# RomanJuranek/waldboost

Measured on AMD Instinct MI355X. Metric: candidate windows/s, 1080p grad_hist pyramid, 128-stage depth-2 cascade, higher is better.
Workload: dtype u8 image, f64/f32 channel arithmetic, f32 scores; 1 GPU; BASELINE configs[1]: 1920x1080 uint8, shrink=2 n_per_oct=8 smooth=1 grad_hist, window (12,12,4), 128-stage depth-2 cascade, 1 image(s)/step/GPU; batch_per_gpu=1, levels=64, windows_per_image=3045278, launch=hipGraph replay per step, only=all, channels_in_hbm=uint8 threshold ranks of the cascade (WB_DTYPE_RANK8), streams=4, pool=4, full=False, warm=1668 untimed steps right before the timed ones (--warm-ms 50), cascade_kernel=model-specialised (hiprtc at model load, 0.9 s incl. cache lookup), collective=none

## Files before the change

### waldboost_amd/csrc/wb_channels.hip

```cpp
#include <stdlib.h>
#include <type_traits>

#include "wb_common.h"

namespace {

struct ChanArgs {
    const void *img;
    const void *oct;
    int64_t img_stride, oct_stride;
    const WbLevel *levels;
    const WbTile *tiles;
    const uint32_t *minmax;
    const WbTap *taps;
    int n_oct;
    void *chn;
    int64_t chn_stride;
    double cs[4], sn[4];
    float chi, clo;
    float c2hi, c2lo;
    double tri[11];
    float gm_eps;
    int src_int;
    int dbg;
    uint8_t *rank;
    int64_t rank_stride;
    const WbTilePatch *patches;
    const uint4 *rank_lut;
    int rank_iters;
    float rank_k[4], rank_b[4];
    int rank_wide;
};

#ifdef WB_CASC_STAMPS
#define WB_CSTAMP_SLOTS 8
#define WB_CSTAMP_WGS (1 << 17)
__device__ unsigned long long g_chan_stamps[WB_CSTAMP_WGS * WB_CSTAMP_SLOTS];
#define WB_CSTAMP(k)                                                                                      \
    do {                                                                                                  \
        unsigned long long _wg = (unsigned long long)blockIdx.y * gridDim.x + blockIdx.x;                 \
        if (threadIdx.x == 0 && _wg < WB_CSTAMP_WGS)                                                      \
            g_chan_stamps[_wg * WB_CSTAMP_SLOTS + (k)] = __builtin_amdgcn_s_memrealtime();                \
    } while (0)
#else
#define WB_CSTAMP(k) do {} while (0)
#endif

#ifndef WB_CHAN_UR
#define WB_CHAN_UR 8
#endif
#ifndef WB_CHAN_S4_BYTES
#define WB_CHAN_S4_BYTES 1
#endif
#ifndef WB_CHAN_S4_WAVES
#define WB_CHAN_S4_WAVES (WB_CHAN_S4_BYTES ? 5 : 3)
#endif
#ifndef WB_CHAN_S4_TV
#define WB_CHAN_S4_TV 30
#endif
typedef WbTap Tap;

__device__ inline double lane_f64(double v, int k) {
    const long long b = __double_as_longlong(v);
    const unsigned lo = (unsigned)__builtin_amdgcn_readlane((int)(unsigned)b, k);
    const unsigned hi = (unsigned)__builtin_amdgcn_readlane((int)(unsigned)(b >> 32), k);
    return __longlong_as_double((long long)(((unsigned long long)hi << 32) | lo));
}

typedef const __attribute__((address_space(3))) unsigned char *LdsBytePtr;
__device__ inline uint8_t lds_byte_apart(const unsigned char *p) {
    LdsBytePtr q = (LdsBytePtr)p;
    asm volatile("" : "+v"(q));
    return *q;
}
typedef const volatile __attribute__((address_space(3))) unsigned char *LdsVolBytePtr;
__device__ __forceinline__ uint8_t lds_byte_vol(const unsigned char *patch, int off) {
    return *((LdsVolBytePtr)patch + off);
}
typedef const volatile __attribute__((address_space(3))) uint16_t *LdsVolU16Ptr;
__device__ __forceinline__ uint32_t lds_u16_vol(const unsigned char *base, int off) {
    return *(LdsVolU16Ptr)((LdsVolBytePtr)base + off);
}

__device__ inline double resample_f64(double v00, double v01, double v10, double v11, const Tap &tr, const Tap &tc) {
    double t = (v00 * tr.w0) * tc.w0;
    t = t + (v01 * tr.w0) * tc.w1;
    t = t + (v10 * tr.w1) * tc.w0;
    t = t + (v11 * tr.w1) * tc.w1;
    return t;
}

template <typename T> struct Src;
template <> struct Src<uint8_t> {
    static constexpr bool kFastResample = true;
    static constexpr float kEps = 2.5e-4f;
    static __device__ bool fast(float v00, float v01, float v10, float v11, float wr0, float wr1, float wc0, float wc1,
                                float &out) {
        float top = __builtin_fmaf(v01, wc1, v00 * wc0), bot = __builtin_fmaf(v11, wc1, v10 * wc0);
        return fast_rows(top, bot, wr0, wr1, out);
    }
    static __device__ bool fast_rows(float top, float bot, float wr0, float wr1, float &out) {
        float t = hold(__builtin_fmaf(bot, wr1, hold(top * wr0)));
        float fl = floorf(t), fr = hold(t - fl);
        out = fl;
        return fabsf(hold(fr - 0.5f)) <= 0.5f - kEps;
    }
    static __device__ __forceinline__ float hold(float v) {
        asm volatile("" : "+v"(v));
        return v;
    }
    static __device__ double lo(uint32_t k) { return (double)k; }
    static __device__ float finish(double t, double mn, double mx, int) {
        t = fmin(fmax(t, mn), mx);
        return (float)(int)t;
    }
    static __device__ bool taps_finite(uint8_t, uint8_t, uint8_t) { return true; }
    static __device__ float hpass(float a, float b, float c) { return __builtin_fmaf(b, 2.0f, a + c); }
    static __device__ float dpass(float lo, float, float hi) { return lo - hi; }
};
template <> struct Src<float> {
    static constexpr bool kFastResample = false;
    static __device__ bool fast(float, float, float, float, float, float, float, float, float &) { return false; }
    static __device__ bool fast_rows(float, float, float, float, float &) { return false; }
    static __device__ double lo(uint32_t k) { return (double)wb_key_f32(k); }
    static __device__ float finish(double t, double mn, double mx, int) {
        const float f = (float)t, lo = (float)mn, hi = (float)mx;
        if (lo != lo || hi != hi) return __builtin_nanf("");
        return f < lo ? lo : (f > hi ? hi : f);
    }
    static __device__ bool taps_finite(float a, float b, float c) { return fabsf(a) < INFINITY && fabsf(b) < INFINITY && fabsf(c) < INFINITY; }
    static __device__ float hpass(float a, float b, float c) {
        return (float)((double)b * 2.0 + ((double)a + (double)c));
    }
    static __device__ float dpass(float lo, float mid, float hi) { return (float)((double)mid * 0.0 + ((double)lo - (double)hi)); }
};

template <> struct Src<double> {
    static constexpr bool kFastResample = false;
    static __device__ bool fast(float, float, float, float, float, float, float, float, float &) { return false; }
    static __device__ bool fast_rows(float, float, float, float, float &) { return false; }
    static __device__ double lo(unsigned long long k) {
        const unsigned long long b = (k >> 63) ? (k & 0x7fffffffffffffffull) : ~k;
        return __longlong_as_double((long long)b);
    }
    static __device__ float finish(double t, double mn, double mx, int src_int) {
        if (mn != mn || mx != mx) return __builtin_nanf("");
        t = t < mn ? mn : (t > mx ? mx : t);
        switch (src_int) {
            case WB_CAST_TRUNC: t = trunc(t); break;
            case WB_CAST_BOOL: t = t != 0.0 ? 1.0 : 0.0; break;
            case WB_CAST_F16: t = wb_round_f16(t); break;
        }
        return (float)t;
    }
    static __device__ bool taps_finite(double a, double b, double c) { return fabs(a) < INFINITY && fabs(b) < INFINITY && fabs(c) < INFINITY; }
    static __device__ float hpass(float a, float b, float c) { return Src<float>::hpass(a, b, c); }
    static __device__ float dpass(float lo, float mid, float hi) { return Src<float>::dpass(lo, mid, hi); }
};

template <typename T> __device__ inline void clip_range(const ChanArgs &a, int b, int oct, double &mn, double &mx) {
    if constexpr (sizeof(T) == 8) {
        const unsigned long long *mm = reinterpret_cast<const unsigned long long *>(a.minmax) + ((int64_t)b * a.n_oct + oct) * 2;
        mn = Src<T>::lo(~mm[0]);
        mx = Src<T>::lo(mm[1]);
    } else {
        const uint32_t *mm = a.minmax + ((int64_t)b * a.n_oct + oct) * 2;
        mn = Src<T>::lo(~mm[0]);
        mx = Src<T>::lo(mm[1]);
    }
}

struct F4 {
    float x, y, z, w;
};

__device__ inline float scalar_only(float v) {
    asm volatile("" : "+v"(v));
    return v;
}

__device__ inline double smooth_top(double a, double b, double c) { return __builtin_fma(2.0, b, a) + c; }
__device__ inline double smooth_mid(double s, double d, double e, double f) {
    return __builtin_fma(2.0, f, __builtin_fma(4.0, e, __builtin_fma(2.0, d, s)));
}
__device__ inline float smooth_bot(double s, double g, double h, double i) { return (float)((__builtin_fma(2.0, h, s + g) + i) * 0.0625); }
__device__ inline float smooth9(double a, double b, double c, double d, double e, double f, double g, double h, double i) {
    return smooth_bot(smooth_mid(smooth_top(a, b, c), d, e, f), g, h, i);
}

__device__ inline void project_f64(float gx, float gy, const ChanArgs &a, float *out) {
    double gxd = (double)gx, gyd = (double)gy;
#pragma unroll
    for (int k = 0; k < 4; ++k) {
        float val = (float)(gxd * a.cs[k] - gyd * a.sn[k]);
        out[k] = fmaxf(fabsf(val), 0.0f);
    }
}

__device__ inline void project_int(float gx, float gy, const ChanArgs &a, float *out) {
    const float d1 = fabsf(gx - gy), d3 = fabsf(gx + gy), ax = fabsf(gx);
    const double g = (double)gx;
    const float tiny = fabsf((float)(g * a.cs[1] - g * a.sn[1]));
    const float o1 = __builtin_fmaf(d1, a.chi, d1 * a.clo), o3 = __builtin_fmaf(d3, a.chi, d3 * a.clo);
    out[0] = ax;
    out[1] = d1 == 0.0f ? tiny : o1;
    out[2] = gy == 0.0f ? __builtin_fmaf(ax, a.c2hi, ax * a.c2lo) : fabsf(gy);
    out[3] = d3 == 0.0f ? tiny : o3;
}

constexpr float kSinHi = 0x1.6a09e6p-1f;
constexpr float kSinLo = (float)(0x1.6a09e667f3bccp-1 - (double)kSinHi);
__device__ inline void project_ordinary(float gx, float gy, const ChanArgs &, float *out) {
    const float d1 = gx - gy, d3 = gx + gy;
    out[0] = fabsf(gx);
    out[1] = fabsf(scalar_only(__builtin_fmaf(d1, kSinHi, scalar_only(d1 * kSinLo))));
    out[2] = fabsf(gy);
    out[3] = fabsf(scalar_only(__builtin_fmaf(d3, kSinHi, scalar_only(d3 * kSinLo))));
}

template <int S_, int TU_, int TV_, bool SMOOTH_, int NT_ = 256> struct TileGeom {
    static constexpr int S = S_, TU = TU_, TV = TV_, NT = NT_, NW = NT_ / 64;
    static constexpr bool SMOOTH = SMOOTH_;
    static constexpr int HS = SMOOTH ? 1 : 0;
    static constexpr int SU = TU + 2 * HS, SV = TV + 2 * HS;
    static constexpr int RH = S * SU + 2, RW = S * SV + 2;
    static constexpr int P = S + 2;
    static constexpr int PROWS = S == 2 ? (TU == 16 ? 74 : 2 * RH - 8) : 2 * RH + 4;
    static constexpr int PPITCH = S == 4 ? 2 * RW + 12 : (S == 2 && TU != 16) ? 256 : ((SU * SV * 16) / PROWS) & ~3;
    static_assert(S == 4 || PROWS * PPITCH <= SU * SV * 16, "the source patch shares the shrunk tile's memory");
    static_assert(PPITCH % 4 == 0, "patch rows are written as dwords");
    static constexpr int SH_BYTES = SU * SV * 16;
    static constexpr int PATCH_BYTES = PROWS * PPITCH;
};

__host__ __device__ inline int reflect_index(int i, int n) {
    const int period = 2 * n;
    i %= period;
    if (i < 0) i += period;
    return i >= n ? period - 1 - i : i;
}

template <bool REFLECT> __host__ __device__ __forceinline__ int tile_coord(int i, int n) {
    if constexpr (REFLECT)
        return reflect_index(i, n);
    else
        return i < 0 ? 0 : (i > n - 1 ? n - 1 : i);
}

template <bool REFLECT> __host__ __device__ __forceinline__ void tile_coord_range(int lo, int hi, int n, int &lo_out, int &hi_out) {
    if constexpr (!REFLECT) {
        lo_out = tile_coord<false>(lo, n);
        hi_out = tile_coord<false>(hi, n);
    } else if (lo >= 0 && hi < n) {
        lo_out = lo;
        hi_out = hi;
    } else if (lo < -n || hi >= 2 * n || (lo < 0 && hi >= n)) {
        lo_out = 0;
        hi_out = n - 1;
    } else if (lo < 0) {
        lo_out = hi < 0 ? -1 - hi : 0;
        hi_out = hi < 0 ? -1 - lo : (hi > -1 - lo ? hi : -1 - lo);
    } else {
        hi_out = lo >= n ? 2 * n - 1 - lo : n - 1;
        lo_out = lo >= n ? 2 * n - 1 - hi : (lo < 2 * n - 1 - hi ? lo : 2 * n - 1 - hi);
    }
}

template <typename G, bool REFLECT>
__host__ __device__ __forceinline__ bool tile_patch_extent(const WbLevel &L, int ry0, int rx0, int rh, int &r_lo, int &c_lo, int &nrow,
                                                           int &nbyte) {
    int yf, yl, xf, xl;
    tile_coord_range<REFLECT>(ry0, ry0 + rh - 1, L.nh, yf, yl);
    tile_coord_range<REFLECT>(rx0, rx0 + G::RW - 1, L.nw, xf, xl);
    const bool ident = (L.src_h == L.nh) && (L.src_w == L.nw);
    const bool strict = !ident && L.src_h > L.nh && L.src_w > L.nw;
    auto first_tap = [](int k, double step) { return (int)floor(((double)k + 0.5) * step - 0.5); };
    r_lo = first_tap(yf, L.sy);
    c_lo = first_tap(xf, L.sx);
    const int r_hi = first_tap(yl, L.sy) + 1, c_hi = first_tap(xl, L.sx) + 1;
    nrow = r_hi - r_lo + 1;
    nbyte = c_hi - c_lo + 1;
    return strict && nrow + 1 <= G::PROWS && nbyte + 8 <= G::PPITCH;
}

template <typename RT, int RW> struct RPitch { static constexpr int value = sizeof(RT) == 1 ? ((RW + 3) & ~3) : RW; };

#ifndef WB_CHAN_RB
#define WB_CHAN_RB 2
#endif
__host__ __device__ constexpr int wb_strip_rows(int rh, int nw) { return WB_CHAN_RB * ((rh + nw * WB_CHAN_RB - 1) / (nw * WB_CHAN_RB)); }

template <typename T, typename G, bool REFLECT = false, typename RT = float>
__device__ __forceinline__ void resample_tile(const ChanArgs &a, const WbLevel &L, const T *src, const double mn,
                                              const double mx, const int ry0, const int rx0, const int rh, RT *R,
                                              unsigned char *uni, float4 *rowtab, const int tid) {
    static_assert(sizeof(RT) == 4 || sizeof(T) == 1, "byte R holds uint8 pixels");
    constexpr int RP = RPitch<RT, G::RW>::value;
    auto rput = [&](int idx, float v) {
        if constexpr (sizeof(RT) == 1) R[idx] = (RT)(int)v; else R[idx] = v;
    };
    constexpr int RH = G::RH, RW = G::RW, PPITCH = G::PPITCH, NT = G::NT, NW = G::NW;
    const Tap *__restrict__ rtap = a.taps + L.tap_off;
    const Tap *__restrict__ ctap = rtap + L.nh;
    constexpr int NCS = RW / 64, MAINW = NCS * 64, LEFT = RW - MAINW;
    const int lane = tid & 63, wave = __builtin_amdgcn_readfirstlane(tid >> 6);
    const bool ident = (L.src_h == L.nh) && (L.src_w == L.nw);
    if constexpr (sizeof(T) == 1) {
        constexpr int RWD = (RW + 3) / 4;
        if (ident && ry0 >= 0 && ry0 + RH <= L.nh && rx0 >= 0 && rx0 + 4 * RWD <= L.nw) {
            static_assert(RW % 2 == 0, "pixel pairs");
            typedef uint32_t __attribute__((aligned(1))) u32u;
            constexpr int NE = RH * RWD, PER = (NE + NT - 1) / NT;
            uint32_t v[PER];
            int at[PER];
#pragma unroll
            for (int i = 0; i < PER; ++i) {
                int e = tid + NT * i;
                e = e < NE ? e : NE - 1;
                const int k = e / RWD, d = e - k * RWD;
                v[i] = *reinterpret_cast<const u32u *>(src + (int64_t)(ry0 + k) * L.src_w + rx0 + 4 * d);
                at[i] = k * RP + 4 * d;
            }
#pragma unroll
            for (int i = 0; i < PER; ++i) {
                if constexpr (sizeof(RT) == 1) {
                    *reinterpret_cast<uint32_t *>(R + at[i]) = v[i];
                } else {
                    float2 *dst = reinterpret_cast<float2 *>(R + at[i]);
                    dst[0] = make_float2((float)(v[i] & 0xffu), (float)((v[i] >> 8) & 0xffu));
                    if (at[i] % RW + 2 < RW) dst[1] = make_float2((float)((v[i] >> 16) & 0xffu), (float)(v[i] >> 24));
                }
            }
            WB_CSTAMP(1);
            WB_CSTAMP(2);
            WB_CSTAMP(3);
            return;
        }
    }
    bool staged = false;
    int r_lo = 0, c_lo = 0;
    Tap tcs[NCS], trl, tleft;
    trl.i0 = trl.i1 = 0; trl.w0 = trl.w1 = 0.0;
    tleft = trl;
#pragma unroll
    for (int c = 0; c < NCS; ++c) tcs[c] = trl;
    if constexpr (sizeof(T) == 1) {
        int nrow, nbyte;
        if (a.patches) {
            const WbTilePatch tp = a.patches[blockIdx.x];
            r_lo = tp.r_lo;
            c_lo = tp.c_lo;
            nrow = tp.rows;
            nbyte = tp.bytes;
            staged = nrow != 0;
        } else {
            staged = tile_patch_extent<G, REFLECT>(L, ry0, rx0, rh, r_lo, c_lo, nrow, nbyte);
            r_lo = __builtin_amdgcn_readfirstlane(r_lo);
            c_lo = __builtin_amdgcn_readfirstlane(c_lo);
            nrow = __builtin_amdgcn_readfirstlane(nrow);
            nbyte = __builtin_amdgcn_readfirstlane(nbyte);
        }
        WB_CSTAMP(1);
#pragma unroll
        for (int c = 0; c < NCS; ++c) {
            const int x = tile_coord<REFLECT>(rx0 + lane + 64 * c, L.nw);
            tcs[c] = ctap[x];
        }
        {
            static_assert(wb_strip_rows(RH, NW) <= 64, "one lane per row of the strip");
            const int RS = wb_strip_rows(rh, NW);
            const int kl = wave * RS + lane;
            const int ly = tile_coord<REFLECT>(ry0 + (kl < rh ? kl : rh - 1), L.nh);
            trl = rtap[ly];
            const int lx = tile_coord<REFLECT>(rx0 + MAINW + (lane < LEFT ? lane : 0), L.nw);
            tleft = ctap[lx];
        }
        if (staged) {
            constexpr int DWP = PPITCH / 4;
            const int ndw = (nbyte + 1 + 3) / 4;
            uint32_t *pw = reinterpret_cast<uint32_t *>(uni);
            constexpr int UR = WB_CHAN_UR;
            const int wv = __builtin_amdgcn_readfirstlane(tid >> 6), ln = tid & 63;
            for (int dw0 = 0; dw0 < ndw; dw0 += 64) {
                int dw = dw0 + ln;
                dw = dw < ndw ? dw : ndw - 1;
                const int voff = 4 * dw;
                const uint64_t origin = reinterpret_cast<uint64_t>(src + (int64_t)r_lo * L.src_w + c_lo);
                const uint64_t origin_u = ((uint64_t)(uint32_t)__builtin_amdgcn_readfirstlane((int)(uint32_t)(origin >> 32)) << 32) |
                                          (uint32_t)__builtin_amdgcn_readfirstlane((int)(uint32_t)origin);
                const __amdgpu_buffer_rsrc_t rsrc = __builtin_amdgcn_make_buffer_rsrc(reinterpret_cast<void *>(origin_u), 0, 0x7fffffff, 0x00020000);
                for (int r0 = wv; r0 < nrow; r0 += NW * UR) {
                    uint32_t v[UR];
                    int rr[UR];
#pragma unroll
                    for (int k = 0; k < UR; ++k) {
                        rr[k] = r0 + NW * k < nrow ? r0 + NW * k : nrow - 1;
                        v[k] = __builtin_amdgcn_raw_buffer_load_b32(rsrc, voff, rr[k] * L.src_w, 0);
                    }
#pragma unroll
                    for (int k = 0; k < UR; ++k) pw[rr[k] * DWP + dw] = v[k];
                }
            }
            {
                const int RS = wb_strip_rows(rh, NW);
                const int kl = wave * RS + lane;
                if (lane < RS && kl < rh) rowtab[kl] = make_float4(__int_as_float((trl.i0 - r_lo) * PPITCH), (float)trl.w0, (float)trl.w1, 0.0f);
            }
            if (LEFT > 0 && tid >= 64 && tid < 64 + LEFT)
                rowtab[RH + tid - 64] = make_float4(__int_as_float(tleft.i0 - c_lo), (float)tleft.w0, (float)tleft.w1, 0.0f);
            __syncthreads();
        }
    }
    WB_CSTAMP(2);
    if (staged) {
        if constexpr (sizeof(T) == 1) {
            const unsigned char *patch = uni;
            int ci0[NCS];
            float wc0f[NCS], wc1f[NCS];
            const Tap (&tc)[NCS] = tcs;
#pragma unroll
            for (int c = 0; c < NCS; ++c) {
                ci0[c] = tc[c].i0 - c_lo;
                wc0f[c] = (float)tc[c].w0;
                wc1f[c] = (float)tc[c].w1;
            }
            constexpr int RB = WB_CHAN_RB;
            constexpr int RSMAX = wb_strip_rows(RH, NW), NPASS = RSMAX / RB;
            const int RS = wb_strip_rows(rh, NW);
            const int k_lo = wave * RS, k_hi = k_lo + RS < rh ? k_lo + RS : rh;
            float hprev[NCS];
            int o_prev = -1;
#pragma unroll
            for (int c = 0; c < NCS; ++c) hprev[c] = 0.0f;
            auto hlerp = [&](uint8_t x0, uint8_t x1, int c) {
                return scalar_only(__builtin_fmaf((float)x1, wc1f[c], scalar_only((float)x0 * wc0f[c])));
            };
            const int rrow = k_lo * RP + lane;
#pragma unroll
            for (int ps = 0; ps < NPASS; ++ps) {
                const int k0 = k_lo + RB * ps;
                if (k0 >= k_hi) break;
                float4 ent[RB];
                int o0[RB], av[RB][NCS];
                bool shared[RB];
                uint8_t b[RB][NCS][4];
#pragma unroll
                for (int rb = 0; rb < RB; ++rb) {
                    int k = k0 + rb;
                    k = k < k_hi ? k : k_hi - 1;
                    ent[rb] = rowtab[k];
                }
#pragma unroll
                for (int rb = 0; rb < RB; ++rb) {
                    o0[rb] = __builtin_amdgcn_readfirstlane(__float_as_int(ent[rb].x));
                    const int o_above = rb == 0 ? o_prev : o0[rb - 1] + PPITCH;
                    shared[rb] = o0[rb] == o_above;
#pragma unroll
                    for (int c = 0; c < NCS; ++c) {
                        av[rb][c] = ci0[c] + o0[rb];
                        b[rb][c][0] = lds_byte_vol(patch, av[rb][c]);
                        b[rb][c][1] = lds_byte_vol(patch, av[rb][c] + 1);
                        b[rb][c][2] = lds_byte_vol(patch, av[rb][c] + PPITCH);
                        b[rb][c][3] = lds_byte_vol(patch, av[rb][c] + PPITCH + 1);
                    }
                }
                float out[RB][NCS];
                bool need[RB][NCS];
                bool redo = false;
#pragma unroll
                for (int rb = 0; rb < RB; ++rb) {
                    float top[NCS];
                    if (shared[rb]) {
#pragma unroll
                        for (int c = 0; c < NCS; ++c) top[c] = hprev[c];
                    } else {
#pragma unroll
                        for (int c = 0; c < NCS; ++c) top[c] = hlerp(b[rb][c][0], b[rb][c][1], c);
                    }
#pragma unroll
                    for (int c = 0; c < NCS; ++c) {
                        const float bot = hlerp(b[rb][c][2], b[rb][c][3], c);
                        hprev[c] = bot;
                        need[rb][c] = !Src<T>::fast_rows(top[c], bot, ent[rb].y, ent[rb].z, out[rb][c]);
                        redo |= need[rb][c];
                    }
                    o_prev = o0[rb] + PPITCH;
                }
                if (__builtin_amdgcn_ballot_w64(redo) != 0) {
#pragma unroll
                    for (int rb = 0; rb < RB; ++rb) {
                        int k = k0 + rb;
                        k = k < k_hi ? k : k_hi - 1;
                        Tap tr;
                        tr.i0 = tr.i1 = 0;
                        tr.w0 = lane_f64(trl.w0, k - k_lo);
                        tr.w1 = lane_f64(trl.w1, k - k_lo);
#pragma unroll
                        for (int c = 0; c < NCS; ++c) {
                            if (need[rb][c])
                                out[rb][c] = Src<T>::finish(resample_f64((double)b[rb][c][0], (double)b[rb][c][1], (double)b[rb][c][2],
                                                                         (double)b[rb][c][3], tr, tc[c]), mn, mx, a.src_int);
                        }
                    }
                }
#pragma unroll
                for (int rb = 0; rb < RB; ++rb) {
                    if (k0 + rb < k_hi) {
#pragma unroll
                        for (int c = 0; c < NCS; ++c) rput(rrow + (RB * ps + rb) * RP + 64 * c, out[rb][c]);
                    }
                }
            }
            if constexpr (LEFT > 0) {
                const int nleft = (k_hi - k_lo) * LEFT;
                for (int p = lane; p < nleft; p += 64) {
                    const int kk = p / LEFT, q = p - kk * LEFT, k = k_lo + kk;
                    const float4 er = rowtab[k], ec = rowtab[RH + q];
                    const int o = __float_as_int(er.x) + __float_as_int(ec.x);
                    const uint8_t a00 = lds_byte_vol(patch, o), a01 = lds_byte_vol(patch, o + 1);
                    const uint8_t a10 = lds_byte_vol(patch, o + PPITCH), a11 = lds_byte_vol(patch, o + PPITCH + 1);
                    float out = 0.0f;
                    if (!Src<T>::fast((float)a00, (float)a01, (float)a10, (float)a11, er.y, er.z, ec.y, ec.z, out)) {
                        const int y = tile_coord<REFLECT>(ry0 + k, L.nh), x = tile_coord<REFLECT>(rx0 + MAINW + q, L.nw);
                        const Tap tr = rtap[y], tcl = ctap[x];
                        out = Src<T>::finish(resample_f64((double)a00, (double)a01, (double)a10, (double)a11, tr, tcl), mn, mx, a.src_int);
                    }
                    rput(k * RP + MAINW + q, out);
                }
            }
        }
    } else
    {
        Tap tc[NCS];
        float wc0f[NCS], wc1f[NCS];
#pragma unroll
        for (int c = 0; c < NCS; ++c) {
            const int x = tile_coord<REFLECT>(rx0 + lane + 64 * c, L.nw);
            tc[c] = ctap[x];
            wc0f[c] = (float)tc[c].w0;
            wc1f[c] = (float)tc[c].w1;
        }
        constexpr int RB = sizeof(T) == 8 ? 2 : 5;
        for (int k0 = wave; k0 < rh; k0 += NW * RB) {
            Tap tr[RB];
            T v00[RB][NCS], v01[RB][NCS], v10[RB][NCS], v11[RB][NCS];
#pragma unroll
            for (int rb = 0; rb < RB; ++rb) {
                int k = k0 + NW * rb;
                k = k < rh ? k : rh - 1;
                const int y = tile_coord<REFLECT>(ry0 + k, L.nh);
                tr[rb] = rtap[__builtin_amdgcn_readfirstlane(y)];
                const T *r0 = src + (int64_t)__builtin_amdgcn_readfirstlane(tr[rb].i0) * L.src_w;
                const T *r1 = src + (int64_t)__builtin_amdgcn_readfirstlane(tr[rb].i1) * L.src_w;
#pragma unroll
                for (int c = 0; c < NCS; ++c) {
                    v00[rb][c] = r0[tc[c].i0];
                    v01[rb][c] = r0[tc[c].i1];
                    v10[rb][c] = r1[tc[c].i0];
                    v11[rb][c] = r1[tc[c].i1];
                }
            }
#pragma unroll
            for (int rb = 0; rb < RB; ++rb) {
                const int k = k0 + NW * rb;
#pragma unroll
                for (int c = 0; c < NCS; ++c) {
                    float out = 0.0f;
                    if (ident && Src<T>::taps_finite(v01[rb][c], v10[rb][c], v11[rb][c])) {
                        out = (mn != mn || mx != mx) ? __builtin_nanf("") : (float)v00[rb][c];
                    } else {
                        bool ok = false;
                        if constexpr (Src<T>::kFastResample)
                            ok = Src<T>::fast((float)v00[rb][c], (float)v01[rb][c], (float)v10[rb][c], (float)v11[rb][c],
                                              (float)tr[rb].w0, (float)tr[rb].w1, wc0f[c], wc1f[c], out);
                        if (!ok)
                            out = Src<T>::finish(resample_f64((double)v00[rb][c], (double)v01[rb][c], (double)v10[rb][c],
                                                              (double)v11[rb][c], tr[rb], tc[c]), mn, mx, a.src_int);
                    }
                    if (k < rh) rput(k * RP + lane + 64 * c, out);
                }
            }
        }
    }
    WB_CSTAMP(3);
    if constexpr (LEFT > 0) {
        for (int p = staged ? rh * LEFT : tid; p < rh * LEFT; p += NT) {
            const int k = p / LEFT, q = MAINW + p - k * LEFT;
            const int y = tile_coord<REFLECT>(ry0 + k, L.nh), x = tile_coord<REFLECT>(rx0 + q, L.nw);
            float out = 0.0f;
            bool ok = false;
            const Tap tr = rtap[y], tc = ctap[x];
            const T *r0 = src + (int64_t)tr.i0 * L.src_w;
            const T *r1 = src + (int64_t)tr.i1 * L.src_w;
            const T a00 = r0[tc.i0], a01 = r0[tc.i1], a10 = r1[tc.i0], a11 = r1[tc.i1];
            ok = ident && Src<T>::taps_finite(a01, a10, a11);
            if (ok) out = (mn != mn || mx != mx) ? __builtin_nanf("") : (float)a00;
            if constexpr (Src<T>::kFastResample)
                if (!ok) ok = Src<T>::fast((float)a00, (float)a01, (float)a10, (float)a11, (float)tr.w0, (float)tr.w1,
                                           (float)tc.w0, (float)tc.w1, out);
            if (!ok) out = Src<T>::finish(resample_f64((double)a00, (double)a01, (double)a10, (double)a11, tr, tc), mn, mx, a.src_int);
            rput(k * RP + q, out);
        }
    }
}

template <typename T, int S, int TU, int TV, bool SMOOTH, bool FAST, int NT>
__global__ __launch_bounds__(NT, sizeof(T) == 8 ? 1
                                 : S == 4  ? (sizeof(T) == 1 ? WB_CHAN_S4_WAVES : 1)
                                 : (S == 2 && sizeof(T) == 1 && SMOOTH && FAST) ? 5
                                                                               : 4) void channels_kernel(ChanArgs a) {
    using G = TileGeom<S, TU, TV, SMOOTH, NT>;
    constexpr int HS = G::HS, SV = G::SV, RH = G::RH, RW = G::RW, P = G::P;
    constexpr int PATCH_BYTES = sizeof(T) == 1 ? G::PATCH_BYTES : 0;
    constexpr int UNI_MIN = G::SH_BYTES > PATCH_BYTES ? G::SH_BYTES : PATCH_BYTES;
    constexpr bool RBYTES = sizeof(T) == 1 && (S == 2 || (S == 4 && WB_CHAN_S4_BYTES));
    constexpr bool LUT_OVER_SH = RBYTES && S == 2;
    constexpr int UNI_LUT = !RBYTES ? 0 : LUT_OVER_SH ? WB_BIN16_LUT_BYTES : ((G::SH_BYTES + 15) & ~15) + WB_BIN16_LUT_BYTES;
    constexpr int UNI_BYTES = UNI_MIN > UNI_LUT ? UNI_MIN : UNI_LUT;
    using RT = typename std::conditional<RBYTES, uint8_t, float>::type;
    constexpr int RP = RPitch<RT, RW>::value;
    constexpr bool LUT_IN_UNI = RBYTES;
    static_assert(WB_BIN16_LUT_BYTES >= WB_BIN_LUT_BYTES, "table sizes");
    constexpr int R_BYTES = LUT_IN_UNI ? RH * RP : (RH * RW * 4 > WB_BIN16_LUT_BYTES ? RH * RW * 4 : WB_BIN16_LUT_BYTES);
    __shared__ __attribute__((aligned(16))) unsigned char Rraw[R_BYTES];
    RT *R = reinterpret_cast<RT *>(Rraw);
    __shared__ __attribute__((aligned(16))) unsigned char uni[UNI_BYTES];
    unsigned char *lut_lds = LUT_OVER_SH ? uni : LUT_IN_UNI ? uni + ((G::SH_BYTES + 15) & ~15) : Rraw;
    __shared__ uint32_t odd_values;
    __shared__ float4 rowtab[sizeof(T) == 1 ? RH + RW % 64 : 1];
    F4 *Sh = reinterpret_cast<F4 *>(uni);
    constexpr bool SEPARABLE = SMOOTH && FAST;
    if (SEPARABLE && threadIdx.x == 0) odd_values = 0;

    const WbTile tile = a.tiles[blockIdx.x];
    const WbLevel L = a.levels[tile.level];
    const int b = blockIdx.y;
    const int tid = threadIdx.x;
    const int u0 = tile.ty * TU, v0 = tile.tx * TV;

    const T *src = (L.oct == 0) ? (const T *)a.img + (int64_t)b * a.img_stride
                                : (const T *)a.oct + (int64_t)b * a.oct_stride + L.src_off;
    double mn, mx;
    clip_range<T>(a, b, L.oct, mn, mx);

    const int ry0 = S * (u0 - HS) - 1, rx0 = S * (v0 - HS) - 1;
    const int vrows = L.u - u0 < TU ? L.u - u0 : TU;
    const int su_need = vrows + 2 * HS, rh_need = S * su_need + 2;
    WB_CSTAMP(0);
    resample_tile<T, G, false, RT>(a, L, src, mn, mx, ry0, rx0, rh_need, R, uni, rowtab, tid);
    __syncthreads();
    WB_CSTAMP(4);
    if (a.dbg & 1) return;

    auto shrunk_pixel = [&](const int ro, const int so) {
        float ch[S][S][4], gxs[S][S], gys[S][S];
        constexpr bool TWO_PASS = FAST && S > 1;
        if constexpr (RBYTES && S == 2) {
            float pt[P][P];
#pragma unroll
            for (int y = 0; y < P; ++y) {
                const uint32_t lo = lds_u16_vol(Rraw, ro + y * RP), hi = lds_u16_vol(Rraw, ro + y * RP + 2);
                pt[y][0] = (float)(lo & 0xffu);
                pt[y][1] = (float)(lo >> 8);
                pt[y][2] = (float)(hi & 0xffu);
                pt[y][3] = (float)(hi >> 8);
            }
            float ex[P][S], dy[S][P];
#pragma unroll
            for (int r = 0; r < P; ++r)
#pragma unroll
                for (int x = 0; x < S; ++x) ex[r][x] = scalar_only(pt[r][x] - pt[r][x + 2]);
#pragma unroll
            for (int y = 0; y < S; ++y)
#pragma unroll
                for (int c = 0; c < P; ++c) dy[y][c] = scalar_only(pt[y][c] - pt[y + 2][c]);
#pragma unroll
            for (int y = 0; y < S; ++y)
#pragma unroll
                for (int x = 0; x < S; ++x) {
                    gxs[y][x] = scalar_only(Src<T>::hpass(ex[y][x], ex[y + 1][x], ex[y + 2][x]));
                    gys[y][x] = scalar_only(Src<T>::hpass(dy[y][x], dy[y][x + 1], dy[y][x + 2]));
                }
        } else {
        float pt[P][P];
        if constexpr (RBYTES) {
            static_assert(P == 6 && RP % 4 == 0, "shrink-4 patch rows");
#pragma unroll
            for (int y = 0; y < P; ++y) {
                const uint32_t *w = reinterpret_cast<const uint32_t *>(R + ro + y * RP);
                const uint32_t w0 = w[0], w1 = w[1];
                pt[y][0] = (float)(w0 & 0xffu);
                pt[y][1] = (float)((w0 >> 8) & 0xffu);
                pt[y][2] = (float)((w0 >> 16) & 0xffu);
                pt[y][3] = (float)(w0 >> 24);
                pt[y][4] = (float)(w1 & 0xffu);
                pt[y][5] = (float)((w1 >> 8) & 0xffu);
            }
        } else {
#pragma unroll
            for (int y = 0; y < P; ++y)
#pragma unroll
                for (int x = 0; x < P; ++x) pt[y][x] = R[ro + y * RP + x];
        }

        float hc[S][P];
        float hr[P][S];
#pragma unroll
        for (int y = 0; y < S; ++y)
#pragma unroll
            for (int x = 0; x < P; ++x) hc[y][x] = scalar_only(Src<T>::hpass(pt[y][x], pt[y + 1][x], pt[y + 2][x]));
#pragma unroll
        for (int y = 0; y < P; ++y)
#pragma unroll
            for (int x = 0; x < S; ++x) hr[y][x] = scalar_only(Src<T>::hpass(pt[y][x], pt[y][x + 1], pt[y][x + 2]));

#pragma unroll
        for (int y = 0; y < S; ++y)
#pragma unroll
            for (int x = 0; x < S; ++x) {
                gxs[y][x] = scalar_only(Src<T>::dpass(hc[y][x], hc[y][x + 1], hc[y][x + 2]));
                gys[y][x] = scalar_only(Src<T>::dpass(hr[y][x], hr[y + 1][x], hr[y + 2][x]));
            }
        }
#pragma unroll
        for (int y = 0; y < S; ++y)
#pragma unroll
            for (int x = 0; x < S; ++x) {
                const float gx = gxs[y][x], gy = gys[y][x];
                if constexpr (TWO_PASS)
                    project_ordinary(gx, gy, a, ch[y][x]);
                else if constexpr (FAST)
                    project_int(gx, gy, a, ch[y][x]);
                else
                    project_f64(gx, gy, a, ch[y][x]);
            }

        float o[4];
        auto pool = [&]() {
#pragma unroll
            for (int k = 0; k < 4; ++k) {
                if constexpr (S == 1) {
                    o[k] = ch[0][0][k];
                } else if constexpr (S == 2) {
                    o[k] = scalar_only(scalar_only(scalar_only(scalar_only(ch[0][0][k] + ch[1][0][k]) + ch[0][1][k]) + ch[1][1][k]) * 0.25f);
                } else {
                    float q[2][2];
#pragma unroll
                    for (int A = 0; A < 2; ++A)
#pragma unroll
                        for (int B = 0; B < 2; ++B)
                            q[A][B] = scalar_only(scalar_only(scalar_only(scalar_only(ch[2 * A][2 * B][k] + ch[2 * A + 1][2 * B][k]) +
                                                                  ch[2 * A][2 * B + 1][k]) + ch[2 * A + 1][2 * B + 1][k]) * 0.25f);
                    o[k] = scalar_only(scalar_only(scalar_only(scalar_only(q[0][0] + q[1][0]) + q[0][1]) + q[1][1]) * 0.25f);
                }
            }
        };
        auto flag_odd = [&]() {
            const uint32_t lo = __float_as_uint(0.125f) - 1u;
            const uint32_t m01 = min(__float_as_uint(o[0]) - 1u, __float_as_uint(o[1]) - 1u);
            const uint32_t m23 = min(__float_as_uint(o[2]) - 1u, __float_as_uint(o[3]) - 1u);
            if (min(m01, m23) < lo) odd_values = 1;
        };
        pool();
        if constexpr (TWO_PASS) {
            if (o[0] != 0.0f && fminf(fminf(o[1], o[2]), o[3]) == 0.0f) {
#pragma unroll
                for (int y = 0; y < S; ++y)
#pragma unroll
                    for (int x = 0; x < S; ++x) project_int(gxs[y][x], gys[y][x], a, ch[y][x]);
                pool();
                if constexpr (SEPARABLE) flag_odd();
            }
        } else if constexpr (SEPARABLE) {
            flag_odd();
        }
        Sh[so] = F4{o[0], o[1], o[2], o[3]};
    };
    constexpr bool ROWMAP = SV >= 64 && SV - 64 <= 8 && NT % 64 == 0;
    if constexpr (ROWMAP) {
        constexpr int NWV = NT / 64, XC = SV - 64;
        const int lane = tid & 63, wave = __builtin_amdgcn_readfirstlane(tid >> 6);
        int ro = S * (wave * RP + lane), so = wave * SV + lane;
#pragma nounroll
        for (int i = wave; i < su_need; i += NWV) {
            shrunk_pixel(ro, so);
            ro += NWV * S * RP;
            so += NWV * SV;
        }
        if constexpr (XC > 0) {
            if (wave == NWV - 1) {
                for (int p = lane; p < su_need * XC; p += 64) {
                    const int i = p / XC, j = 64 + p - i * XC;
                    shrunk_pixel(S * (i * RP + j), i * SV + j);
                }
            }
        }
    } else {
        for (int p = tid; p < su_need * SV; p += NT) {
            const int i = p / SV, j = p - i * SV;
            shrunk_pixel(S * (i * RP + j), p);
        }
    }
    constexpr int LUT_VECS = WB_BIN_LUT_BYTES / 16, LUT16_VECS = WB_BIN16_LUT_BYTES / 16;
    auto ranks_wide_tag = [](const ChanArgs &aa) { return aa.rank != nullptr && aa.rank_wide != 0; };
    static_assert(LUT_VECS == 768 && NT == 256, "three vectors per thread");
    const bool ranks = a.rank != nullptr;
    uint4 lut0 = make_uint4(0, 0, 0, 0), lut1 = lut0, lut2 = lut0, lut3 = lut0, lut4 = lut0;
    const bool wide_lut = ranks_wide_tag(a);
    if (ranks) {
        lut0 = a.rank_lut[tid];
        lut1 = a.rank_lut[tid + 256];
        lut2 = a.rank_lut[tid + 512];
        if (wide_lut && !LUT_OVER_SH) {
            lut3 = a.rank_lut[tid + 768];
            lut4 = a.rank_lut[tid + 1024];
        }
    }
    static_assert(LUT16_VECS == 1280, "five vectors per thread");
    auto park_tables = [&]() {
        uint4 *lut = reinterpret_cast<uint4 *>(lut_lds);
        lut[tid] = lut0;
        lut[tid + 256] = lut1;
        lut[tid + 512] = lut2;
        if (wide_lut) {
            if constexpr (LUT_OVER_SH) {
                lut3 = a.rank_lut[tid + 768];
                lut4 = a.rank_lut[tid + 1024];
            }
            lut[tid + 768] = lut3;
            lut[tid + 1024] = lut4;
        }
    };
    __syncthreads();
    if (!LUT_OVER_SH && ranks) park_tables();
    WB_CSTAMP(5);

    if (a.dbg & 2) return;
    constexpr bool WHOLE = TU * TV % NT == 0 && NT % TV == 0;
    constexpr int RPT = WHOLE ? TU * TV / NT : 1;
    static_assert(WHOLE || TU * TV <= NT, "one output per thread");
    float *out = reinterpret_cast<float *>(a.chn) + (int64_t)b * a.chn_stride + L.chn_off;
    const int j = tid % TV, i0 = (tid / TV) * RPT;
    const int sv = v0 + j;
    float o[RPT][4];
    const bool live = WHOLE ? (TV != 64 || u0 + __builtin_amdgcn_readfirstlane(i0) < L.u) : i0 < TU;
#pragma unroll
    for (int y = 0; y < RPT; ++y) o[y][0] = o[y][1] = o[y][2] = o[y][3] = 0.0f;
    if (!live) {
    } else if constexpr (SMOOTH) {
        if (SEPARABLE && odd_values == 0) {
            double s[3][2];
            float s32[3][2];
#pragma unroll
            for (int y = 0; y < RPT + 2; ++y) {
                const F4 c0 = Sh[(i0 + y) * SV + j], c1 = Sh[(i0 + y) * SV + j + 1], c2 = Sh[(i0 + y) * SV + j + 2];
                const float a0[4] = {c0.x, c0.y, c0.z, c0.w}, a1[4] = {c1.x, c1.y, c1.z, c1.w}, a2[4] = {c2.x, c2.y, c2.z, c2.w};
#pragma unroll
                for (int h = 0; h < 2; ++h) {
                    s32[y % 3][h] = __builtin_fmaf(2.0f, a1[2 * h], a0[2 * h]) + a2[2 * h];
                    s[y % 3][h] = __builtin_fma(2.0, (double)a1[2 * h + 1], (double)a0[2 * h + 1]) + (double)a2[2 * h + 1];
                }
                if (y >= 2) {
#pragma unroll
                    for (int h = 0; h < 2; ++h) {
                        o[y - 2][2 * h] = (__builtin_fmaf(2.0f, s32[(y - 1) % 3][h], s32[(y - 2) % 3][h]) + s32[y % 3][h]) * 0.0625f;
                        o[y - 2][2 * h + 1] = (float)((__builtin_fma(2.0, s[(y - 1) % 3][h], s[(y - 2) % 3][h]) + s[y % 3][h]) * 0.0625);
                    }
                }
            }
        } else {
            double s[RPT][4];
#pragma unroll
            for (int r = 0; r < RPT + 2; ++r) {
                __builtin_amdgcn_sched_barrier(0);
                const F4 c0 = Sh[(i0 + r) * SV + j], c1 = Sh[(i0 + r) * SV + j + 1], c2 = Sh[(i0 + r) * SV + j + 2];
                const float a0[4] = {c0.x, c0.y, c0.z, c0.w}, a1[4] = {c1.x, c1.y, c1.z, c1.w}, a2[4] = {c2.x, c2.y, c2.z, c2.w};
#pragma unroll
                for (int k = 0; k < 4; ++k) {
                    const double v0 = a0[k], v1 = a1[k], v2 = a2[k];
                    if (r >= 2) o[r - 2][k] = smooth_bot(s[r - 2][k], v0, v1, v2);
                    if (r >= 1 && r - 1 < RPT) s[r - 1][k] = smooth_mid(s[r - 1][k], v0, v1, v2);
                    if (r < RPT) s[r][k] = smooth_top(v0, v1, v2);
                }
            }
        }
    } else {
#pragma unroll
        for (int y = 0; y < RPT; ++y) {
            F4 c = Sh[(i0 + y) * SV + j];
            o[y][0] = c.x; o[y][1] = c.y; o[y][2] = c.z; o[y][3] = c.w;
        }
    }
    if (LUT_OVER_SH && ranks) {
        __syncthreads();
        park_tables();
    }
    WB_CSTAMP(6);
#pragma unroll
    for (int y = 0; y < RPT; ++y) {
        const int su = u0 + i0 + y;
        if ((!WHOLE && !live) || su >= L.u || sv >= L.v || (a.dbg & 4)) continue;
        if (SMOOTH && (su == 0 || sv == 0 || su == L.u - 1 || sv == L.v - 1)) o[y][0] = o[y][1] = o[y][2] = o[y][3] = 0.0f;
        if (a.chn) {
            float4 *dst = reinterpret_cast<float4 *>(out + ((int64_t)su * L.v + sv) * 4);
            *dst = make_float4(o[y][0], o[y][1], o[y][2], o[y][3]);
        }
    }
    if (ranks) {
        __syncthreads();
        const float *Sthr = reinterpret_cast<const float *>(lut_lds);
        const int K = a.rank_iters;
        auto rank_pixels = [&](auto wide_tag) {
            constexpr bool WIDE = decltype(wide_tag)::value;
            constexpr int SLOTS = WIDE ? WB_BIN16_SLOTS : WB_BIN_SLOTS, CELLS = WIDE ? WB_BIN16_CELLS : WB_BIN_CELLS;
            const uint8_t *base8 = reinterpret_cast<const uint8_t *>(lut_lds) + 4 * SLOTS * 4;
            const uint16_t *base16 = reinterpret_cast<const uint16_t *>(base8);
            uint32_t r[RPT][4];
            if (live) {
#pragma unroll
                for (int y = 0; y < RPT; ++y)
#pragma unroll
                    for (int k = 0; k < 4; ++k) {
                        const uint32_t cell = wb_bin_cell(o[y][k], a.rank_k[k], a.rank_b[k], (float)(CELLS - 1));
                        r[y][k] = WIDE ? (uint32_t)base16[k * CELLS + cell] : (uint32_t)base8[k * CELLS + cell];
                    }
                if (K <= 2) {
#pragma unroll
                    for (int y = 0; y < RPT; ++y)
#pragma unroll
                        for (int k = 0; k < 4; ++k) {
                            const float *sp = Sthr + k * SLOTS + r[y][k];
                            const float s0 = sp[0], s1 = sp[1];
                            r[y][k] += (o[y][k] > s0 ? 1u : 0u) + (o[y][k] > s1 ? 1u : 0u);
                        }
                } else if (WIDE && K <= 4) {
#pragma unroll
                    for (int y = 0; y < RPT; ++y)
#pragma unroll
                        for (int k = 0; k < 4; ++k) {
                            const float *sp = Sthr + k * SLOTS + r[y][k];
                            const float s0 = sp[0], s1 = sp[1], s2 = sp[2], s3 = sp[3];
                            r[y][k] += (o[y][k] > s0 ? 1u : 0u) + (o[y][k] > s1 ? 1u : 0u) + (o[y][k] > s2 ? 1u : 0u) + (o[y][k] > s3 ? 1u : 0u);
                        }
                } else {
                    for (int i = 0; i < K; ++i) {
#pragma unroll
                        for (int y = 0; y < RPT; ++y)
#pragma unroll
                            for (int k = 0; k < 4; ++k) r[y][k] += o[y][k] > Sthr[k * SLOTS + r[y][k]] ? 1u : 0u;
                    }
                }
            }
#pragma unroll
            for (int y = 0; y < RPT; ++y) {
                const int su = u0 + i0 + y;
                if (!live || su >= L.u || sv >= L.v || (a.dbg & 4)) continue;
                uint32_t rk[4];
#pragma unroll
                for (int k = 0; k < 4; ++k) {
                    rk[k] = r[y][k];
                    if constexpr (sizeof(T) != 1) rk[k] = o[y][k] != o[y][k] ? (WIDE ? 65535u : 255u) : rk[k];
                }
                if constexpr (WIDE) {
                    uint2 *rout = reinterpret_cast<uint2 *>(reinterpret_cast<uint16_t *>(a.rank) + ((int64_t)b * a.rank_stride + L.chn_off));
                    rout[(int64_t)su * L.v + sv] = make_uint2(rk[0] | (rk[1] << 16), rk[2] | (rk[3] << 16));
                } else {
                    uint32_t *rout = reinterpret_cast<uint32_t *>(a.rank + (int64_t)b * a.rank_stride + L.chn_off);
                    rout[(int64_t)su * L.v + sv] = rk[0] | (rk[1] << 8) | (rk[2] << 16) | (rk[3] << 24);
                }
            }
        };
        if (a.rank_wide)
            rank_pixels(std::true_type{});
        else
            rank_pixels(std::false_type{});
    }
    WB_CSTAMP(7);
}

template <int S, int TU, int TV, bool SMOOTH, int NCH>
__global__ __launch_bounds__(256) void channels_u1_kernel(ChanArgs a) {
    using T = uint8_t;
    using G = TileGeom<S, TU, TV, SMOOTH>;
    constexpr int HS = G::HS, SU = G::SU, SV = G::SV, RH = G::RH, RW = G::RW, P = G::P;
    constexpr int UNI_BYTES = G::SH_BYTES > G::PATCH_BYTES ? G::SH_BYTES : G::PATCH_BYTES;
    __shared__ float R[RH * RW];
    __shared__ __attribute__((aligned(16))) unsigned char uni[UNI_BYTES];
    __shared__ float4 rowtab[RH + RW % 64];
    uint32_t *Sh = reinterpret_cast<uint32_t *>(uni);

    const WbTile tile = a.tiles[blockIdx.x];
    const WbLevel L = a.levels[tile.level];
    const int b = blockIdx.y;
    const int tid = threadIdx.x;
    const int u0 = tile.ty * TU, v0 = tile.tx * TV;
    const T *src = (L.oct == 0) ? (const T *)a.img + (int64_t)b * a.img_stride
                                : (const T *)a.oct + (int64_t)b * a.oct_stride + L.src_off;
    double mn, mx;
    clip_range<T>(a, b, L.oct, mn, mx);
    const int ry0 = S * (u0 - HS) - 1, rx0 = S * (v0 - HS) - 1;
    resample_tile<T, G>(a, L, src, mn, mx, ry0, rx0, RH, R, uni, rowtab, tid);
    __syncthreads();
    if (a.dbg & 1) return;

    for (int p = tid; p < SU * SV; p += 256) {
        const int i = p / SV, j = p - i * SV;
        float pt[P][P];
#pragma unroll
        for (int y = 0; y < P; ++y)
#pragma unroll
            for (int x = 0; x < P; ++x) pt[y][x] = R[(S * i + y) * RW + (S * j + x)];
        float hc[S][P], hr[P][S];
#pragma unroll
        for (int y = 0; y < S; ++y)
#pragma unroll
            for (int x = 0; x < P; ++x) hc[y][x] = scalar_only(Src<T>::hpass(pt[y][x], pt[y + 1][x], pt[y + 2][x]));
#pragma unroll
        for (int y = 0; y < P; ++y)
#pragma unroll
            for (int x = 0; x < S; ++x) hr[y][x] = scalar_only(Src<T>::hpass(pt[y][x], pt[y][x + 1], pt[y][x + 2]));
        const int by0 = ry0 + S * i + 1, bx0 = rx0 + S * j + 1;
        const bool on_border = by0 <= 0 || bx0 <= 0 || by0 + S - 1 >= L.nh - 1 || bx0 + S - 1 >= L.nw - 1;
        int ch[S][S][NCH];
#pragma unroll
        for (int y = 0; y < S; ++y)
#pragma unroll
            for (int x = 0; x < S; ++x) {
                float dx = scalar_only(hc[y][x + 2] - hc[y][x]);
                float dy = scalar_only(hr[y + 2][x] - hr[y][x]);
                if (on_border) {
                    const int gy = by0 + y, gx = bx0 + x;
                    if (gy <= 0 || gx <= 0 || gy >= L.nh - 1 || gx >= L.nw - 1) dx = dy = 0.0f;
                }
                if constexpr (NCH == 4) {
                    ch[y][x][0] = (int)(uint32_t)fabsf(dx) >> 2;
                    ch[y][x][1] = (int)(uint32_t)fabsf(dx - dy) >> 3;
                    ch[y][x][2] = (int)(uint32_t)fabsf(dy) >> 2;
                    ch[y][x][3] = (int)(uint32_t)fabsf(dx + dy) >> 3;
                } else {
                    ch[y][x][0] = (int)(uint32_t)fmaxf(fabsf(dx), fabsf(dy)) >> 2;
                }
            }
        uint32_t o = 0;
#pragma unroll
        for (int k = 0; k < NCH; ++k) {
            int v;
            if constexpr (S == 1) {
                v = ch[0][0][k];
            } else if constexpr (S == 2) {
                v = ((ch[0][0][k] + ch[1][0][k] + ch[0][1][k] + ch[1][1][k]) & 255) >> 2;
            } else {
                int q[2][2];
#pragma unroll
                for (int A = 0; A < 2; ++A)
#pragma unroll
                    for (int B = 0; B < 2; ++B)
                        q[A][B] = ((ch[2 * A][2 * B][k] + ch[2 * A + 1][2 * B][k] + ch[2 * A][2 * B + 1][k] +
                                    ch[2 * A + 1][2 * B + 1][k]) & 255) >> 2;
                v = ((q[0][0] + q[1][0] + q[0][1] + q[1][1]) & 255) >> 2;
            }
            o |= (uint32_t)v << (8 * k);
        }
        Sh[p] = o;
    }
    __syncthreads();
    if (a.dbg & 2) return;

    constexpr int RPT = TU * TV / 256;
    static_assert(TU * TV % 256 == 0 && 256 % TV == 0, "tile must split into whole thread strips");
    uint8_t *out = reinterpret_cast<uint8_t *>(a.chn) + (int64_t)b * a.chn_stride + L.chn_off;
    const int j = tid % TV, i0 = (tid / TV) * RPT;
    const int sv = v0 + j;
    uint32_t o[RPT];
    if constexpr (SMOOTH) {
        uint32_t w[RPT + 2][3];
#pragma unroll
        for (int y = 0; y < RPT + 2; ++y)
#pragma unroll
            for (int x = 0; x < 3; ++x) w[y][x] = Sh[(i0 + y) * SV + (j + x)];
#pragma unroll
        for (int y = 0; y < RPT; ++y) {
            o[y] = 0;
#pragma unroll
            for (int k = 0; k < NCH; ++k) {
                auto at = [&](int yy, int xx) { return (int)((w[y + yy][xx] >> (8 * k)) & 255u); };
                const int sum = at(0, 0) + 2 * at(0, 1) + at(0, 2) + 2 * at(1, 0) + 4 * at(1, 1) + 2 * at(1, 2) +
                                at(2, 0) + 2 * at(2, 1) + at(2, 2);
                o[y] |= (uint32_t)(sum >> 4) << (8 * k);
            }
        }
    } else {
#pragma unroll
        for (int y = 0; y < RPT; ++y) o[y] = Sh[(i0 + y) * SV + j];
    }
#pragma unroll
    for (int y = 0; y < RPT; ++y) {
        const int su = u0 + i0 + y;
        if (su >= L.u || sv >= L.v || (a.dbg & 4)) continue;
        if (SMOOTH && (su == 0 || sv == 0 || su == L.u - 1 || sv == L.v - 1)) o[y] = 0;
        const int64_t at = (int64_t)su * L.v + sv;
        if constexpr (NCH == 4)
            reinterpret_cast<uint32_t *>(out)[at] = o[y];
        else
// ... 596 lines not shown
```

Measured before the change: 59.66 billion windows/s.

## Reuse overlapping patch rows across contiguous row strips in shrunk-pixel gradient pass

For byte-resampled S=2 tiles, each wave now takes a contiguous block of shrunk rows instead of striding by the wave count. Within that block it keeps the horizontal diffs and smoothed rows of the overlapping patch rows in registers, so each step loads and converts only the new rows. It also replaces the float-to-int byte store in resample with a magic-number add and bit cast. The cost is more register pressure from the unrolled per-wave row loop, and wave load is less even when su_need does not divide evenly across waves.

```diff
diff --git a/waldboost_amd/csrc/wb_channels.hip b/waldboost_amd/csrc/wb_channels.hip
--- a/waldboost_amd/csrc/wb_channels.hip
+++ b/waldboost_amd/csrc/wb_channels.hip
@@ -290,14 +290,19 @@
 #endif
 __host__ __device__ constexpr int wb_strip_rows(int rh, int nw) { return WB_CHAN_RB * ((rh + nw * WB_CHAN_RB - 1) / (nw * WB_CHAN_RB)); }
 
-template <typename T, typename G, bool REFLECT = false, typename RT = float>
+template <typename T, typename G, bool REFLECT = false, typename RT = float, bool RADD = false>
 __device__ __forceinline__ void resample_tile(const ChanArgs &a, const WbLevel &L, const T *src, const double mn,
                                               const double mx, const int ry0, const int rx0, const int rh, RT *R,
                                               unsigned char *uni, float4 *rowtab, const int tid) {
     static_assert(sizeof(RT) == 4 || sizeof(T) == 1, "byte R holds uint8 pixels");
     constexpr int RP = RPitch<RT, G::RW>::value;
     auto rput = [&](int idx, float v) {
-        if constexpr (sizeof(RT) == 1) R[idx] = (RT)(int)v; else R[idx] = v;
+        if constexpr (sizeof(RT) == 1 && RADD)
+            R[idx] = (RT)__float_as_uint(scalar_only(v + 8388608.0f));
+        else if constexpr (sizeof(RT) == 1)
+            R[idx] = (RT)(int)v;
+        else
+            R[idx] = v;
     };
     constexpr int RH = G::RH, RW = G::RW, PPITCH = G::PPITCH, NT = G::NT, NW = G::NW;
     const Tap *__restrict__ rtap = a.taps + L.tap_off;
@@ -647,15 +652,18 @@
     const int vrows = L.u - u0 < TU ? L.u - u0 : TU;
     const int su_need = vrows + 2 * HS, rh_need = S * su_need + 2;
     WB_CSTAMP(0);
-    resample_tile<T, G, false, RT>(a, L, src, mn, mx, ry0, rx0, rh_need, R, uni, rowtab, tid);
+    resample_tile<T, G, false, RT, RBYTES && S == 2>(a, L, src, mn, mx, ry0, rx0, rh_need, R, uni, rowtab, tid);
     __syncthreads();
     WB_CSTAMP(4);
     if (a.dbg & 1) return;
 
-    auto shrunk_pixel = [&](const int ro, const int so) {
+    struct OwnPatch {};
+    auto shrunk_pixel = [&](const int ro, const int so, auto grads) {
         float ch[S][S][4], gxs[S][S], gys[S][S];
         constexpr bool TWO_PASS = FAST && S > 1;
-        if constexpr (RBYTES && S == 2) {
+        if constexpr (!std::is_same<decltype(grads), OwnPatch>::value) {
+            grads(gxs, gys);
+        } else if constexpr (RBYTES && S == 2) {
             float pt[P][P];
 #pragma unroll
             for (int y = 0; y < P; ++y) {
@@ -780,25 +788,75 @@
     if constexpr (ROWMAP) {
         constexpr int NWV = NT / 64, XC = SV - 64;
         const int lane = tid & 63, wave = __builtin_amdgcn_readfirstlane(tid >> 6);
-        int ro = S * (wave * RP + lane), so = wave * SV + lane;
+        if constexpr (RBYTES && S == 2) {
+            constexpr int MAXR = (G::SU + NWV - 1) / NWV;
+            const int q = su_need / NWV, rem = su_need % NWV;
+            const int n_w = q + (wave < rem ? 1 : 0), i_w = wave * q + (wave < rem ? wave : rem);
+            const int ro = S * (i_w * RP + lane), so = i_w * SV + lane;
+            auto patch_row = [&](const uint32_t lo, const uint32_t hi, float (&e)[S], float (&h)[S]) {
+                const float p0 = scalar_only((float)(lo & 0xffu)), p1 = scalar_only((float)(lo >> 8));
+                const float p2 = scalar_only((float)(hi & 0xffu)), p3 = scalar_only((float)(hi >> 8));
+                e[0] = scalar_only(p0 - p2);
+                e[1] = scalar_only(p1 - p3);
+                h[0] = scalar_only(Src<T>::hpass(p0, p1, p2));
+                h[1] = scalar_only(Src<T>::hpass(p1, p2, p3));
+            };
+            float ex[P][S], hr[P][S];
+#pragma unroll
+            for (int r = 0; r < MAXR; ++r) {
+                if (r >= n_w) break;
+                const int o = ro + r * S * RP;
+                const int y0 = r == 0 ? 0 : S;
+                uint32_t lo[P], hi[P];
+#pragma unroll
+                for (int y = 0; y < P; ++y) {
+                    if (y < y0) continue;
+                    lo[y] = lds_u16_vol(Rraw, o + y * RP);
+                    hi[y] = lds_u16_vol(Rraw, o + y * RP + 2);
+                }
+#pragma unroll
+                for (int y = 0; y < P; ++y) {
+                    if (y >= y0) {
+                        patch_row(lo[y], hi[y], ex[y], hr[y]);
+                    } else {
+#pragma unroll
+                        for (int x = 0; x < S; ++x) {
+                            ex[y][x] = ex[y + S][x];
+                            hr[y][x] = hr[y + S][x];
+                        }
+                    }
+                }
+                shrunk_pixel(o, so + r * SV, [&](float (&gxs)[S][S], float (&gys)[S][S]) {
+#pragma unroll
+                    for (int y = 0; y < S; ++y)
+#pragma unroll
+                        for (int x = 0; x < S; ++x) {
+                            gxs[y][x] = scalar_only(Src<T>::hpass(ex[y][x], ex[y + 1][x], ex[y + 2][x]));
+                            gys[y][x] = scalar_only(hr[y][x] - hr[y + 2][x]);
+                        }
+                });
+            }
+        } else {
+            int ro = S * (wave * RP + lane), so = wave * SV + lane;
 #pragma nounroll
-        for (int i = wave; i < su_need; i += NWV) {
-            shrunk_pixel(ro, so);
-            ro += NWV * S * RP;
-            so += NWV * SV;
+            for (int i = wave; i < su_need; i += NWV) {
+                shrunk_pixel(ro, so, OwnPatch{});
+                ro += NWV * S * RP;
+                so += NWV * SV;
+            }
         }
         if constexpr (XC > 0) {
             if (wave == NWV - 1) {
                 for (int p = lane; p < su_need * XC; p += 64) {
                     const int i = p / XC, j = 64 + p - i * XC;
-                    shrunk_pixel(S * (i * RP + j), i * SV + j);
+                    shrunk_pixel(S * (i * RP + j), i * SV + j, OwnPatch{});
                 }
             }
         }
     } else {
         for (int p = tid; p < su_need * SV; p += NT) {
             const int i = p / SV, j = p - i * SV;
-            shrunk_pixel(S * (i * RP + j), p);
+            shrunk_pixel(S * (i * RP + j), p, OwnPatch{});
         }
     }
     constexpr int LUT_VECS = WB_BIN_LUT_BYTES / 16, LUT16_VECS = WB_BIN16_LUT_BYTES / 16;
```

Result: faster. 61.80 billion windows/s (median of 6 runs) (+3.6%).
